# eazuooz/RayTracinginOneWeekendinCUDA

Hardware: AMD Instinct MI355X
Metric: Msamples/s (pixels x spp / s), whole job (higher is better)
Workload: dtype f64; 1 GPU; C2 Book-1 final random-spheres, HittableList world (no BVH), 1200x800x500spp x50 bounces; frames_in_flight=1, width=1200, height=800, spp=500, max_depth=50, seed=1984, variant=strict, rng=XORWOW (cuRAND device-API semantics), one sequence per pixel

## Files before the change

raytracinginoneweekendincuda_amd/csrc/device_scene.cpp:

```cpp
#include <hip/hip_runtime.h>

#include <cstdio>
#include <cmath>
#include <cstring>
#include <initializer_list>
#include <map>
#include <mutex>
#include <string>
#include <type_traits>
#include <utility>
#include <vector>

#include "../../include/rtow.h"
#include "device_arena.h"
#include "film_rows.h"
#include "launch_plan.h"
#include "primary_cull_rule.h"
#include "render_iface.h"
#include "scene_host.h"

namespace rtow {

static int hip_fail(hipError_t e, const char *what)
{
// ... 1004 lines not shown
    if (rc != RT_OK) {
        const std::string why = rt_last_error();
        hipStreamSynchronize(stream);
        mark_done(f);
        f.seeded = false;
        set_error(why);
        return rc;
    }
    f.last_samples = (uint64_t)f.geometry.n_pixels * (uint64_t)p->samples_per_pixel;
    f.last_variant = p->variant;
    f.last_adaptive = f.adaptive;
    f.last_direct = direct != nullptr;
    f.rendered = true;
    return RT_OK;
}

int rt_render_launch(rt_scene *scene, rt_film *film, const rt_render_params *p)
{
    if (int rc = frame_launch_check(scene, film, p, "rt_render_launch")) return rc;
    return launch_frame(scene, film, p, nullptr);
}

int rt_render_launch_direct(rt_scene *scene, rt_film *film, const rt_render_params *p, const rt_film_direct_params *direct)
{
    const std::string who = "rt_render_launch_direct";
    if (int rc = frame_launch_check(scene, film, p, who)) return rc;
    if (!direct) return fail(RT_ERR_INVALID, who + ": direct is NULL");
    if (direct->strategy != 0 && direct->strategy != 1) return fail(RT_ERR_INVALID, who + ": strategy must be 0 (uniform) or 1 (by area and brightness)");
    for (int32_t word : direct->reserved)
        if (word != 0) return fail(RT_ERR_INVALID, who + ": reserved must be 0");
    return launch_frame(scene, film, p, direct);
}

int rt_film_last_direct_stats(rt_film *film, rt_film_direct_stats *out)
{
    if (!film || !out) return fail(RT_ERR_INVALID, "rt_film_last_direct_stats: null argument");
    const FilmImpl &f = *F(film);
    if (!f.has_direct_stats) return fail(RT_ERR_STATE, "rt_film_last_direct_stats: no direct launch of this film has been finished");
    *out = f.direct_stats;
    return RT_OK;
}

void rt_film_direct_abi_sizes(uint32_t out2[2])
{
    out2[0] = (uint32_t)sizeof(rt_film_direct_params);
    out2[1] = (uint32_t)sizeof(rt_film_direct_stats);
}

#if RT_PHASES
static void print_phases(const FilmImpl &f)
{
    const unsigned long long *c = f.host_counters;
    const char *name[24] = {"node step", "leaf test", "shade", "refill", "  group/instance", "  medium", "  primitive", "",
                            "    record+xforms", "    box", "    sub-BVH", "    other geometry", "between walks again", "limited node pass", "node visits (lanes)", "",
                            "box pass", "medium pass / between walks", "object pass", "primitive pass", "  hit record", "  scatter",
                            "  next camera ray", "  pixel done"};
    if (is_sphere_list_kernel(f.last_kernel.kind)) {
        name[0] = "scan, pixel-parallel";
        name[1] = "scan, cooperative";
        name[12] = name[13] = "";
        const double passes = (double)c[96 + 0], groups = (double)c[96 + 12], taken = (double)c[64 + 12];
        if (groups > 0) {
            std::fprintf(stderr, "survivors: %.0f passes, %.2f groups of 4 per pass, groups taken f = %.4f\n", passes, groups / passes, taken / groups);
            std::fprintf(stderr, "survivors: spheres with a passing lane per taken group %.3f, lane appends per pass %.1f, lanes behind per pass %.2f\n",
                         (double)c[32 + 12] / taken, (double)c[96 + 13] / passes, (double)c[64 + 13] / passes);
            std::fprintf(stderr, "survivors: drains per pass %.2f, drain iterations (wave max of count) per pass %.2f, drain cycles %.1f %% of the "
                         "pixel-parallel scan's (%.0f of %.0f per pass)\n", (double)c[96 + 15] / passes, (double)c[64 + 15] / passes,
                         100.0 * c[32 + 13] / c[32 + 0], (double)c[32 + 13] / passes, (double)c[32 + 0] / passes);
        }
        name[19] = "";
        if (c[96 + 19])
            std::fprintf(stderr, "camera rays: %llu pixel-parallel passes, %.2f live lanes per pass, %.2f of them with a camera ray (depth 0): share %.4f\n",
                         c[96 + 19], (double)c[64 + 19] / c[96 + 19], (double)c[32 + 19] / c[96 + 19], (double)c[32 + 19] / (double)c[64 + 19]);
        name[23] = "";
        if (c[96 + 23])
            std::fprintf(stderr, "primary: %llu rounds, %.2f fresh lanes per round, %.2f list entries tested per round (%.2f per lane), %.0f cycles per round "
                         "(%.1f %% of wave time)\n", c[96 + 23], (double)c[64 + 23] / c[96 + 23], (double)c[32 + 15] / c[96 + 23],
                         (double)c[32 + 15] / (double)c[64 + 23], (double)c[32 + 23] / c[96 + 23], 100.0 * c[32 + 23] / (double)c[7]);
        name[14] = name[7] = "";
        if (c[96 + 7])
            std::fprintf(stderr, "window: %llu windowed passes (%llu windowed runs), %.2f trips scanned per pass in them, %.2f ranges per pass, %.0f cycles "
                         "of window computation per pass\n", c[96 + 7] * 16ull, c[96 + 14] * 16ull, (double)c[64 + 14] / c[96 + 7], (double)c[64 + 7] / c[96 + 7],
                         (double)c[32 + 14] / c[96 + 7]);
        name[16] = name[17] = name[18] = "";
        const double gp = (double)c[96 + 16];
        if (gp > 0) {
            std::fprintf(stderr, "grouped: %.0f passes through the filter, %.2f rays per pass, exact-test blocks executed per pass %.2f\n", gp,
                         (double)c[64 + 16] / gp, (double)c[32 + 16] / gp);
            std::fprintf(stderr, "grouped: survivors (lanes tested) per pass %.2f, largest per-lane count per pass %.2f, drains per pass %.2f\n",
                         (double)c[32 + 17] / gp, (double)c[64 + 17] / gp, (double)c[96 + 17] / gp);
            std::fprintf(stderr, "grouped: cycles per pass: filter %.0f, exact tests %.0f (%.1f %% and %.1f %% of the cooperative scans' %.0f)\n",
                         (double)c[64 + 18] / gp, (double)c[32 + 18] / gp, 100.0 * c[64 + 18] / c[32 + 1], 100.0 * c[32 + 18] / c[32 + 1],
                         (double)c[32 + 1] / (double)c[96 + 1]);
        }
    }
    const double total = (double)c[7];
    for (int k = 0; k < 24; k++)
        if (name[k][0] && c[96 + k])
            std::fprintf(stderr, "phase %-20s: %5.1f %% of wave time, %10llu passes, %5.1f lanes/pass, %7.0f cycles/pass\n", name[k],
                         100.0 * c[32 + k] / total, c[96 + k], (double)c[64 + k] / c[96 + k], (double)c[32 + k] / c[96 + k]);
}
#endif

int rt_render_finish(rt_scene *scene, rt_film *film, rt_render_stats *stats)
{
    (void)scene;
    if (!film) return fail(RT_ERR_INVALID, "rt_render_finish: null film");
    FilmImpl &f = *F(film);
    if (!f.in_flight) return fail(RT_ERR_STATE, "rt_render_finish: nothing launched");
    if (int rc = select_device(f.device)) return rc;
    const hipError_t waited = hipEventSynchronize(f.ev[3]);
    if (waited != hipSuccess && f.last_stream) hipStreamSynchronize(f.last_stream);
    mark_done(f);
    if (waited != hipSuccess) return hip_fail(waited, "hipEventSynchronize(render finished)");
    if (f.last_direct) {
        f.direct_stats = rt_film_direct_stats{f.host_counters[kShadowCounterWord], f.host_counters[kShadowCounterWord + 1], (uint32_t)f.last_direct_scratch, 0u};
        f.has_direct_stats = true;
    }
    if (stats) {
        std::memset(stats, 0, sizeof *stats);
        float ms_seed = 0, ms_render = 0;
        HIP_TRY(hipEventElapsedTime(&ms_seed, f.ev[0], f.ev[1]));
        HIP_TRY(hipEventElapsedTime(&ms_render, f.ev[1], f.ev[2]));
        const unsigned long long rays = f.host_counters[0];
#if RT_PHASES
        print_phases(f);
#endif
        stats->samples = f.last_adaptive ? (uint64_t)f.host_counters[2] : f.last_samples;
        stats->rays = rays;
        stats->seconds_seed = ms_seed * 1e-3;
        stats->seconds_render = ms_render * 1e-3;
        stats->pixels = f.geometry.n_pixels;
        stats->rows = (uint32_t)f.geometry.rows_owned;
        stats->kernel_vgprs = (uint32_t)f.last_kernel.vgprs;
        stats->lds_bytes = (uint32_t)f.last_kernel.lds_bytes;
        stats->kernel_kind = (uint32_t)f.last_kernel.kind;
        stats->pixels_per_wave = (uint32_t)f.last_plan.pixels_per_wave;
    }
    return RT_OK;
}

int rt_film_download(rt_film *film, double *frame_full, int width, int height)
{
    if (!film || !frame_full) return fail(RT_ERR_INVALID, "rt_film_download: null argument");
    FilmImpl &f = *F(film);
    if (width != f.geometry.width || height != f.geometry.height) return fail(RT_ERR_INVALID, "rt_film_download: frame size mismatch");
    if (int rc = select_device(f.device)) return rc;
    return download_rows(f, f.pixels, 3, false, frame_full);
}

int rt_film_set_adaptive(rt_film *film, const rt_adaptive_params *params)
{
    if (!film) return fail(RT_ERR_INVALID, "rt_film_set_adaptive: null film");
    FilmImpl &f = *F(film);
    if (f.in_flight) return fail(RT_ERR_STATE, "rt_film_set_adaptive: a render is in flight");
    if (params && !rule_in_range(*params))
        return fail(RT_ERR_INVALID, "rt_film_set_adaptive: needs min_samples >= 2, check_interval >= 1, noise_threshold >= 0, luminance_floor > 0");
    f.adaptive = params != nullptr;
    if (params) f.rule = to_rule(*params);
    return RT_OK;
}

int rt_film_download_sample_counts(rt_film *film, uint32_t *counts_full, int width, int height)
{
    if (!film || !counts_full) return fail(RT_ERR_INVALID, "rt_film_download_sample_counts: null argument");
    FilmImpl &f = *F(film);
    if (width != f.geometry.width || height != f.geometry.height) return fail(RT_ERR_INVALID, "rt_film_download_sample_counts: frame size mismatch");
    if (f.in_flight) return fail(RT_ERR_STATE, "rt_film_download_sample_counts: a render is in flight");
    if (int rc = select_device(f.device)) return rc;
    if (f.rendered && f.last_adaptive) return download_rows(f, f.ad_n, 1, true, counts_full);
    const std::vector<uint32_t> compact((size_t)f.geometry.n_pixels, f.rendered ? (uint32_t)f.frame_spp : 0u);
    scatter_owned_rows(compact.data(), 1, width, height, f.stripe_rows, f.rank, f.world_size, true, counts_full);
    return RT_OK;
}

int rt_film_download_probe_costs(rt_film *film, uint32_t *costs_full, int width, int height)
// ... 959 lines not shown
```

raytracinginoneweekendincuda_amd/csrc/render.hip:

```cpp
#include <hip/hip_runtime.h>

#include <cfloat>
#include <cstddef>
#include <cstdint>
#include <type_traits>

#include "flat_scene.h"
#include "launch_plan.h"
#include "primary_cull_rule.h"
#include "scan_window_rule.h"
#include "render_iface.h"
#include "rng.h"

#ifndef RT_STRICT
#define RT_STRICT 1
#endif
#ifndef RT_GROUP
#define RT_GROUP 0
#endif
#ifndef RT_ADAPT
#define RT_ADAPT 0
#endif
#ifndef RT_FEATURES
#define RT_FEATURES 0
// ... 324 lines not shown
            accept = aa_inside<P, Q>(f.wa, f.qp, f.qq, f.ku, f.kv, r, t[k]);                                            \
        }                                                                                                               \
        const bool take = live && accept;                                                                               \
        closest = take ? t[k] : closest;                                                                                \
        ref_best = take ? make_ref(REF_QUAD, quad_first + k) : ref_best;                                                \
        any = any || take;                                                                                              \
    }
    RT_BOX_FACE(0, 0, 1)
    RT_BOX_FACE(1, 2, 1)
    RT_BOX_FACE(2, 0, 1)
    RT_BOX_FACE(3, 2, 1)
    RT_BOX_FACE(4, 0, 2)
    RT_BOX_FACE(5, 0, 2)
#undef RT_BOX_FACE
    t_best = closest;
    return any;
}

DEV Vec msphere_center(const MSphereGeom &g, double tm, bool unit_time = false)
{
    double frac = unit_time ? tm : (tm - g.t0) / g.dt;
    return mk(g.c0x, g.c0y, g.c0z) + frac * mk(g.dcx, g.dcy, g.dcz);
}

DEV bool prim_test(const DeviceScene &sc, uint32_t ref, const Ray &r, double a, double tmin, double tmax, double &t)
{
    uint32_t idx = ref & kRefIndexMask;
    switch (ref >> kRefShift) {
    case REF_SPHERE: {
        SphereGeom g = sc.lds_spheres_tab != kNone ? lds_row<SphereGeom>(sc.lds_spheres_tab, idx) : const_row(sc.spheres, idx);
        return sphere_test(r.o - mk(g.cx, g.cy, g.cz), r.d, a, g.r2, tmin, tmax, t);
    }
    case REF_MSPHERE: {
        MSphereGeom g = const_row(sc.mspheres, idx);
        return sphere_test(r.o - msphere_center(g, r.tm, (sc.flags & SCENE_MS_UNIT_TIME) != 0), r.d, a, g.r2, tmin, tmax, t);
    }
    default: {
        return quad_test_at(sc, idx, r, tmin, tmax, t);
    }
    }
}

#ifndef RT_PHASES
#define RT_PHASES 0
#endif
#if RT_PHASES && RT_LANE_UNIT
#undef RT_PHASES
#define RT_PHASES 0
#endif
#if RT_PHASES
#define PH_BEGIN() const unsigned long long ph_t0 = __builtin_readcyclecounter()
#define PH_END(k, cond)                                                   \
    do {                                                                  \
        ph.t[k] += __builtin_readcyclecounter() - ph_t0;                  \
        ph.l[k] += (unsigned long long)__popcll(__ballot(cond));          \
        ph.n[k] += 1ull;                                                  \
    } while (0)
struct PhaseSums {
    unsigned long long t[24], l[24], n[24];
};
#define PH_ARG , PhaseSums &ph
#define PH_PASS , ph
#define PH_SUB_BEGIN() const unsigned long long ph_s0 = __builtin_readcyclecounter()
#define PH_COUNT(k) do { ph.l[k] += 1024ull; ph.n[k] += 1024ull; } while (0)
#define PH_SUB_END(k)                                                                              \
    do {                                                                                           \
        const unsigned long long ph_pc = (unsigned long long)__popcll(__ballot(true));             \
        ph.t[k] += (__builtin_readcyclecounter() - ph_s0) * 1024ull / ph_pc;                       \
        ph.l[k] += 1024ull;                                                                        \
        ph.n[k] += 1024ull / ph_pc;                                                                \
    } while (0)
#else
#define PH_BEGIN() do { } while (0)
#define PH_END(k, cond) do { } while (0)
#define PH_ARG
#define PH_PASS
#define PH_SUB_BEGIN() do { } while (0)
#endif
#if RT_PHASES
struct ScanSums {
    uint32_t groups, taken, spheres, appends, behind;
    uint32_t drains, drain_iters, drain_cycles;
    uint32_t win_runs, win_trips, win_ranges, win_cycles;
};
#define SS_ARG , ScanSums &ss
#define SS_PASS , ss
struct GroupedSums {
    uint32_t rays, tests, survivors, lane_max;
    uint32_t drains, filter_cycles, test_cycles;
};
#define GS_ARG , GroupedSums &gs
#define GS_PASS , gs
#else
#define SS_ARG
#define SS_PASS
#define GS_ARG
#define GS_PASS
#define PH_COUNT(k) do { } while (0)
#define PH_SUB_END(k) do { } while (0)
#endif
DEV Vec affine_rows(const DeviceScene &sc, uint32_t row, Vec p)
{
    const Xform r0 = get_xform(sc, row), r1 = get_xform(sc, row + 1), r2 = get_xform(sc, row + 2);
    return mk(((r0.a * p.x) + (r0.b * p.y)) + (r0.c * p.z), ((r1.a * p.x) + (r1.b * p.y)) + (r1.c * p.z), ((r2.a * p.x) + (r2.b * p.y)) + (r2.c * p.z));
}
DEV void affine_to_local(const DeviceScene &sc, uint32_t head, const Xform &x, Ray &lr)
{
    lr.o = affine_rows(sc, head + 4, lr.o - mk(x.a, x.b, x.c));
    lr.d = affine_rows(sc, head + 4, lr.d);
}
DEV void affine_to_world(const DeviceScene &sc, uint32_t head, Vec &p, Vec &n)
{
    const Xform t = get_xform(sc, head);
    p = affine_rows(sc, head + 1, p) + mk(t.a, t.b, t.c);
    const Xform i0 = get_xform(sc, head + 4), i1 = get_xform(sc, head + 5), i2 = get_xform(sc, head + 6);
    const Vec m = mk(((i0.a * n.x) + (i1.a * n.y)) + (i2.a * n.z), ((i0.b * n.x) + (i1.b * n.y)) + (i2.b * n.z), ((i0.c * n.x) + (i1.c * n.y)) + (i2.c * n.z));
    n = (1.0 / sqrt(length_sq(m))) * m;
}
struct MovingPose { Vec l[3], i[3], t; };
struct VecPair { Vec a, b; };
DEV MovingPose moving_pose(const Xform *rows, double tm)
{
    const Xform t0 = rows[0], dt = rows[4], key = rows[8];
    double s = (tm - key.a) / key.b;
    s = fmin(fmax(s, 0.0), 1.0);
    MovingPose m;
    for (uint32_t r = 0; r < 3; r++) {
        const Xform a = rows[1 + r], d = rows[5 + r];
        m.l[r] = mk(a.a + (s * d.a), a.b + (s * d.b), a.c + (s * d.c));
    }
    m.t = mk(t0.a + (s * dt.a), t0.b + (s * dt.b), t0.c + (s * dt.c));
    const Vec l0 = m.l[0], l1 = m.l[1], l2 = m.l[2];
    const double c00 = (l1.y * l2.z) - (l1.z * l2.y), c01 = (l1.z * l2.x) - (l1.x * l2.z), c02 = (l1.x * l2.y) - (l1.y * l2.x);
    const double c10 = (l0.z * l2.y) - (l0.y * l2.z), c11 = (l0.x * l2.z) - (l0.z * l2.x), c12 = (l0.y * l2.x) - (l0.x * l2.y);
    const double c20 = (l0.y * l1.z) - (l0.z * l1.y), c21 = (l0.z * l1.x) - (l0.x * l1.z), c22 = (l0.x * l1.y) - (l0.y * l1.x);
    const double det = ((l0.x * c00) + (l0.y * c01)) + (l0.z * c02);
    m.i[0] = mk(c00 / det, c10 / det, c20 / det);
    m.i[1] = mk(c01 / det, c11 / det, c21 / det);
    m.i[2] = mk(c02 / det, c12 / det, c22 / det);
    return m;
}
DEV Vec pose_rows(const Vec (&m)[3], Vec p)
{
    return mk(((m[0].x * p.x) + (m[0].y * p.y)) + (m[0].z * p.z), ((m[1].x * p.x) + (m[1].y * p.y)) + (m[1].z * p.z), ((m[2].x * p.x) + (m[2].y * p.y)) + (m[2].z * p.z));
}
DEV VecPair moving_local(const Xform *rows, double tm, Vec o, Vec d)
{
    const MovingPose m = moving_pose(rows, tm);
    return VecPair{pose_rows(m.i, o - m.t), pose_rows(m.i, d)};
}
DEV VecPair moving_world(const Xform *rows, double tm, Vec p, Vec n)
{
    const MovingPose m = moving_pose(rows, tm);
    const Vec v = mk(((m.i[0].x * n.x) + (m.i[1].x * n.y)) + (m.i[2].x * n.z), ((m.i[0].y * n.x) + (m.i[1].y * n.y)) + (m.i[2].y * n.z), ((m.i[0].z * n.x) + (m.i[1].z * n.y)) + (m.i[2].z * n.z));
    return VecPair{pose_rows(m.l, p) + m.t, (1.0 / sqrt(length_sq(v))) * v};
}
DEV const Xform *xform_rows(const DeviceScene &sc, uint32_t i)
{
    return (sc.lds_xforms != kNone ? reinterpret_cast<const Xform *>(lds_raw + sc.lds_xforms) : sc.xforms) + i;
}
DEV void moving_to_local(const DeviceScene &sc, uint32_t head, Ray &lr)
{
    const VecPair v = moving_local(xform_rows(sc, head), lr.tm, lr.o, lr.d);
    lr.o = v.a;
    lr.d = v.b;
}
// ... 1273 lines not shown
DEV ScanWindowSeg load_scan_window(const ScanWindowSeg *table, uint32_t k)
{
    const RT_CONST uint32_t *p = (const RT_CONST uint32_t *)(uintptr_t)(table + k);
    return ScanWindowSeg{p[0], __builtin_bit_cast(float, p[1]), __builtin_bit_cast(float, p[2]), p[3]};
}
DEV ScanTripSpan load_scan_span(const DeviceScene &sc, uint32_t t)
{
    if (sc.lds_scan_spans != kNone && sc.lds_scan_spans != 0u) {
        const v2f v = *(const RT_LDS v2f *)(lds_raw + sc.lds_scan_spans + t * (uint32_t)sizeof(ScanTripSpan));
        return ScanTripSpan{v.x, v.y};
    }
    return reinterpret_cast<const ScanTripSpan *>(sc.scan_segments + 2u * sc.n_scan_segments)[t];
}
template <int CTRL, int ROW_MASK>
DEV void fmin_step(float &x, float &y)
{
    const float ox = __builtin_bit_cast(float, __builtin_amdgcn_update_dpp(__builtin_bit_cast(int, x), __builtin_bit_cast(int, x), CTRL, ROW_MASK, 0xf, false));
    const float oy = __builtin_bit_cast(float, __builtin_amdgcn_update_dpp(__builtin_bit_cast(int, y), __builtin_bit_cast(int, y), CTRL, ROW_MASK, 0xf, false));
    x = __builtin_fminf(x, ox);
    y = __builtin_fminf(y, oy);
}
DEV void wave_fmin2(float &x, float &y)
{
    fmin_step<0xB1, 0xf>(x, y);
    fmin_step<0x4E, 0xf>(x, y);
    fmin_step<0x114, 0xf>(x, y);
    fmin_step<0x118, 0xf>(x, y);
    fmin_step<0x142, 0xa>(x, y);
    fmin_step<0x143, 0xc>(x, y);
    x = __builtin_bit_cast(float, __builtin_amdgcn_readlane(__builtin_bit_cast(int, x), 63));
    y = __builtin_bit_cast(float, __builtin_amdgcn_readlane(__builtin_bit_cast(int, y), 63));
}
template <bool ROWS_IN_LDS, bool WINDOWS>
DEV bool scan_filtered32(const DeviceScene &sc, bool live, uint32_t planes_off, uint32_t n_padded, uint16_t *queue, uint32_t lane,
                         const Ray &r, double tmin, double tmax, HitInfo &best SS_ARG)
{
    static_assert(kFilterTrip == 2 * kScanTripPairs && kScanAheadPairs == 2, "one trip = four pairs in two halves; set A of the next trip is read ahead");
    constexpr uint32_t kPairBytes = (uint32_t)sizeof(SphereScanPair), kTripBytes = kScanTripPairs * kPairBytes;
    const SphereScanPair *__restrict__ rows = sc.sphere_scan32;
    const ScanSegment *__restrict__ segments = sc.scan_segments;
    const SphereGeom *__restrict__ spheres = sc.spheres;
    const uint32_t n_segments = sc.n_scan_segments;
    const double a = dot(r.d, r.d);
    ScanRayPairs f = scan_ray_pairs(scan_ray32(r, a, sc.scan_reach32));
    if constexpr (WINDOWS)
        if (!live) f.nt = v2f{-__builtin_inff(), -__builtin_inff()};
    double closest = tmax;
    uint32_t best_k = kNone, count = 0;
    if (n_segments) {
        SphereScanPair a0 = load_scan_pair(rows, 0u, 0u), a1 = load_scan_pair(rows, 0u, kPairBytes);
        uint32_t off = 0, end = 0;
        for (uint32_t seg = 0; seg != n_segments; seg++) {
            const ScanSegment sg = load_scan_segment(segments, seg);
            end = (sg.first_trip + sg.n_trips) * kTripBytes;
            if (sg.axis == kScanAxisNone) {
                do scan_trip<false, ROWS_IN_LDS>(rows, spheres, off, end, a0, a1, f, f.ux, f.nt, planes_off, n_padded, queue, lane, count, r, a, tmin, closest, best_k SS_PASS);
                while (off != end);
            } else {
                const uint32_t seg_end = end;
                bool windowed = false;
                float x0 = 0.0f, x1 = 0.0f;
                uint32_t chunk = sg.first_trip;
                unsigned long long need = 0;
                if constexpr (WINDOWS) {
                    const ScanWindowSeg *windows = reinterpret_cast<const ScanWindowSeg *>(segments + n_segments);
                    const ScanWindowSeg ws = load_scan_window(windows, seg);
                    const uint32_t window_axis = ws.axis;
                    windowed = window_axis != kScanAxisNone;
                    if (windowed) {
#if RT_PHASES
                        const unsigned long long ss_w0 = __builtin_readcyclecounter();
#endif
                        const bool in_run = lane < sg.n_trips;
                        ScanTripSpan sp{0.0f, 0.0f};
                        if (in_run) sp = load_scan_span(sc, sg.first_trip + lane);
                        float e0 = __builtin_inff(), e1 = __builtin_inff();
                        if (live) {
                            const double oa = sg.axis == 0u ? r.o.x : (sg.axis == 1u ? r.o.y : r.o.z), da = sg.axis == 0u ? r.d.x : (sg.axis == 1u ? r.d.y : r.d.z);
                            const double ow = window_axis == 0u ? r.o.x : (window_axis == 1u ? r.o.y : r.o.z), dw = window_axis == 0u ? r.d.x : (window_axis == 1u ? r.d.y : r.d.z);
                            const ScanExtent ex = scan_window_extent(oa, da, ow, dw, __builtin_fabs(r.o.x) + __builtin_fabs(r.o.y) + __builtin_fabs(r.o.z), a, sc.scan_reach32, (double)ws.slab_lo, (double)ws.slab_hi);
                            e0 = (float)ex.lo;
                            e1 = -(float)ex.hi;
                        }
                        wave_fmin2(e0, e1);
                        x0 = e0;
                        x1 = -e1;
                        need = scan_window_fill(__ballot(in_run && scan_window_needs(sp.lo, sp.hi, x0, x1)));
#if RT_PHASES
                        asm volatile("" ::"s"(x0), "s"(x1));
                        ss.win_cycles += (uint32_t)(__builtin_readcyclecounter() - ss_w0);
                        ss.win_runs++;
#endif
                    }
                }
                if (sg.axis == 0u) { scan_swap(f.ux, f.uy); scan_swap(f.px, f.py); }
                if (sg.axis == 2u) { scan_swap(f.uz, f.uy); scan_swap(f.pz, f.py); }
                const v2f c = {sg.c, sg.c};
                v2f s0 = c * f.uy, l0 = __builtin_elementwise_fma(f.py, c, f.nt);
                if (!windowed) {
                    do scan_trip<true, ROWS_IN_LDS>(rows, spheres, off, end, a0, a1, f, s0, l0, planes_off, n_padded, queue, lane, count, r, a, tmin, closest, best_k SS_PASS);
                    while (off != end);
                } else {
                    for (;;) {
                        while (!need && (chunk + 64u) * kTripBytes < seg_end) {
                            chunk += 64u;
                            const uint32_t n = seg_end / kTripBytes - chunk;
                            bool mine = false;
                            if (lane < n) {
                                const ScanTripSpan sp = load_scan_span(sc, chunk + lane);
                                mine = scan_window_needs(sp.lo, sp.hi, x0, x1);
                            }
                            need = scan_window_fill(__ballot(mine));
                        }
                        if (!need) break;
                        const uint32_t first = (uint32_t)__builtin_ctzll(need);
                        const unsigned long long behind = ~(need >> first);
                        const uint32_t len = behind ? (uint32_t)__builtin_ctzll(behind) : 64u - first;
                        need &= need + (1ull << first);
                        const uint32_t start = (chunk + first) * kTripBytes;
                        if (start != off) {
                            off = start;
                            a0 = load_scan_pair(rows, off, 0u);
                            a1 = load_scan_pair(rows, off, kPairBytes);
                        }
                        end = start + len * kTripBytes;
#if RT_PHASES
                        ss.win_ranges++;
                        ss.win_trips += len;
#endif
                        do scan_trip<true, ROWS_IN_LDS>(rows, spheres, off, end, a0, a1, f, s0, l0, planes_off, n_padded, queue, lane, count, r, a, tmin, closest, best_k SS_PASS);
                        while (off != end);
                    }
                }
                if (off != seg_end) {
                    off = seg_end;
                    a0 = load_scan_pair(rows, off, 0u);
                    a1 = load_scan_pair(rows, off, kPairBytes);
                }
                if (sg.axis == 0u) { scan_swap(f.ux, f.uy); scan_swap(f.px, f.py); }
                if (sg.axis == 2u) { scan_swap(f.uz, f.uy); scan_swap(f.pz, f.py); }
            }
        }
    }
    drain_filtered<ROWS_IN_LDS>(spheres, planes_off, n_padded, queue, lane, count, r, a, tmin, closest, best_k SS_PASS);
    if (best_k == kNone) return false;
    best.t = closest;
    best.ref = make_ref(REF_SPHERE, best_k);
    best.obj = kNone;
    return true;
}

template <bool ROWS_IN_LDS>
DEV bool scan_filtered(const DeviceScene &sc, uint32_t planes_off, uint32_t n_padded, uint16_t *queue, uint32_t lane, const Ray &r, double tmin,
                       double tmax, HitInfo &best SS_ARG)
{
    const SphereScanRow *__restrict__ rows = sc.sphere_scan;
    const SphereGeom *__restrict__ spheres = sc.spheres;
    const uint32_t n = sc.n_spheres;
    const uint32_t n8 = n & ~7u;
    const double a = dot(r.d, r.d);
    const ScanRay f = scan_ray(r, a, sc.scan_reach);
    double closest = tmax;
    uint32_t best_k = kNone, count = 0;
    SphereScanRow a0{}, a1{}, a2{}, a3{};
    if (n8) {
        a0 = load_scan_row(rows, 0); a1 = load_scan_row(rows, 1);
        a2 = load_scan_row(rows, 2); a3 = load_scan_row(rows, 3);
    }
    for (uint32_t k0 = 0; k0 < n8; k0 += 8) {
        scan_rows_arrived(a0, a1, a2, a3);
        const SphereScanRow b0 = load_scan_row(rows, k0 + 4), b1 = load_scan_row(rows, k0 + 5);
        const SphereScanRow b2 = load_scan_row(rows, k0 + 6), b3 = load_scan_row(rows, k0 + 7);
        filter_four(a0, a1, a2, a3, k0, f, queue, lane, count);
        const uint32_t kn = (k0 + 8 < n8) ? k0 + 8 : k0;
// ... 127 lines not shown
                    const double cx = sv.plane(0, k), cy = sv.plane(1, k), cz = sv.plane(2, k);
                    const double fs = filter_s(f, cx, cy, cz);
                    q[u] = filter_q(f, fs, cx, cy, cz);
                    pass[u] = q[u] > sv.plane(4, k);
                }
#pragma unroll
                for (int u = 0; u < 4; u++) {
                    const uint32_t k = base + 64u * u + lane;
                    if (k < sv.n && pass[u]) {
                        double t;
                        if (sphere_test(r.o - mk(sv.plane(0, k), sv.plane(1, k), sv.plane(2, k)), r.d, a, sv.plane(3, k), tmin, bt, t)) {
                            bt = t;
                            bk = k;
                        }
                    }
                }
            }
        } else if (sv.in_lds) {
            for (uint32_t base = 0; base < sv.n_padded; base += 256u) {
                double b[4], c[4], disc[4];
#pragma unroll
                for (int u = 0; u < 4; u++) {
                    uint32_t k = base + 64u * u + lane;
                    k = k < sv.n_padded ? k : sv.n_padded - 1u;
                    Vec oc = r.o - mk(sv.plane(0, k), sv.plane(1, k), sv.plane(2, k));
                    b[u] = dot(oc, r.d);
                    c[u] = dot(oc, oc) - sv.plane(3, k);
                    disc[u] = b[u] * b[u] - a * c[u];
                }
#pragma unroll
                for (int u = 0; u < 4; u++) {
                    const uint32_t k = base + 64u * u + lane;
                    if (k < sv.n && disc[u] > 0.0 && !(b[u] > 0.0 && c[u] > 0.0)) {
                        double t;
                        if (sphere_roots(b[u], disc[u], a, tmin, bt, t)) {
                            bt = t;
                            bk = k;
                        }
                    }
                }
            }
        } else {
            for (uint32_t k = lane; k < sv.n; k += 64u) {
                SphereGeom g = sv.global[k];
                Vec oc = r.o - mk(g.cx, g.cy, g.cz);
                double b = dot(oc, r.d);
                double c = dot(oc, oc) - g.r2;
                double disc = b * b - a * c;
                if (disc > 0.0 && !(b > 0.0 && c > 0.0)) {
                    double t;
                    if (sphere_roots(b, disc, a, tmin, bt, t)) {
                        bt = t;
                        bk = k;
                    }
                }
            }
        }
        wave_min(bt, bk);
        if ((int)lane == src) {
            hit = bk != kNone;
            best.t = bt;
            best.ref = make_ref(REF_SPHERE, bk);
            best.obj = kNone;
        }
    }
}

DEV int lane_read(int v, int src_lane) { return __builtin_amdgcn_ds_bpermute(src_lane << 2, v); }
DEV double lane_read(double x, int src_lane)
{
    int lo = lane_read(__double2loint(x), src_lane);
    int hi = lane_read(__double2hiint(x), src_lane);
    return __hiloint2double(hi, lo);
}
DEV void min_with_lane(double &t, uint32_t &k, int partner)
{
    double ot = lane_read(t, partner);
    uint32_t ok = (uint32_t)lane_read((int)k, partner);
    bool take = (ot < t) || (ot == t && ok < k);
    t = take ? ot : t;
    k = take ? ok : k;
}

DEV void scan_grouped(const SphereView &sv, uint32_t lane, unsigned long long todo, const Ray &ray, double tmin, double tmax,
                      HitInfo &best, bool &hit GS_ARG)
{
    const int L = __popcll(todo);
    int log2m = 0;
    while ((1 << log2m) < L) log2m++;
    const int log2g = 6 - log2m;
    const uint32_t g = 1u << log2g;
    const uint32_t q = lane >> log2g, s = lane & (g - 1u);
    int owner = todo ? __ffsll((long long)todo) - 1 : (int)lane;
    {
        unsigned long long m = todo;
        for (int r = 0; r < L; r++) {
            const int src = __ffsll((long long)m) - 1;
            m &= m - 1;
            owner = q == (uint32_t)r ? src : owner;
        }
    }
    Ray r;
    r.o = mk(lane_read(ray.o.x, owner), lane_read(ray.o.y, owner), lane_read(ray.o.z, owner));
    r.d = mk(lane_read(ray.d.x, owner), lane_read(ray.d.y, owner), lane_read(ray.d.z, owner));
    const double a = dot(r.d, r.d);
    double bt = tmax;
    uint32_t bk = kNone;
    if (!sv.exact && sv.pairs_off) {
        const ScanRayPairs f = scan_ray_pairs(scan_ray32(r, a, sv.reach32));
        const uint32_t n_pairs = sv.n_padded / 2u;
        const v4f *rows = reinterpret_cast<const v4f *>(lds_raw + sv.pairs_off);
#if RT_PHASES
        uint32_t gs_mine = 0;
        gs.rays = (uint32_t)L;
#endif
        for (uint32_t base = 0; base < n_pairs; base += 2u * g) {
            v2f fs[2], fq[2], fk[2];
#if RT_PHASES
            const unsigned long long gs_t0 = __builtin_readcyclecounter();
#endif
#pragma unroll
            for (int h = 0; h < 2; h++) {
                uint32_t j = base + g * h + s;
                j = j < n_pairs ? j : n_pairs - 1u;
                const v4f lo = rows[j], hi = rows[n_pairs + j];
                const v2f cx = {lo.x, lo.y}, cy = {lo.z, lo.w}, cz = {hi.x, hi.y};
                fk[h] = v2f{hi.z, hi.w};
                fs[h] = __builtin_elementwise_fma(cz, f.uz, __builtin_elementwise_fma(cy, f.uy, cx * f.ux));
                fq[h] = __builtin_elementwise_fma(fs[h], fs[h], __builtin_elementwise_fma(f.pz, cz, __builtin_elementwise_fma(f.py, cy, __builtin_elementwise_fma(f.px, cx, f.nt))));
            }
            const float sv4[4] = {fs[0].x, fs[0].y, fs[1].x, fs[1].y}, qv4[4] = {fq[0].x, fq[0].y, fq[1].x, fq[1].y};
            const float kv4[4] = {fk[0].x, fk[0].y, fk[1].x, fk[1].y};
#if RT_PHASES
            const unsigned long long gs_t1 = __builtin_readcyclecounter();
#pragma unroll
            for (int u = 0; u < 4; u++) {
                const bool tested = 2u * (base + g * (uint32_t)(u >> 1) + s) + (uint32_t)(u & 1) < sv.n && qv4[u] > kv4[u];
                const unsigned long long m = __ballot(tested);
                gs.tests += m ? 1u : 0u;
                gs.survivors += (uint32_t)__popcll(m);
                gs_mine += tested ? 1u : 0u;
            }
            const unsigned long long gs_t2 = __builtin_readcyclecounter();
            gs.filter_cycles += (uint32_t)(gs_t1 - gs_t0);
#endif
#pragma unroll
            for (int u = 0; u < 4; u++) {
                const uint32_t k = 2u * (base + g * (uint32_t)(u >> 1) + s) + (uint32_t)(u & 1);
                if (k < sv.n && qv4[u] > kv4[u]) {
                    const float bu = f.od - sv4[u];
                    const bool behind = bu > f.root_m && __builtin_fmaf(bu, bu, kv4[u] - qv4[u]) > 0.0f;
                    double t;
                    if (!behind && sphere_test(r.o - mk(sv.plane(0, k), sv.plane(1, k), sv.plane(2, k)), r.d, a, sv.plane(3, k), tmin, bt, t)) {
                        bt = t;
                        bk = k;
                    }
                }
            }
#if RT_PHASES
            asm volatile("" ::"v"(bt), "v"(bk));
            gs.test_cycles += (uint32_t)(__builtin_readcyclecounter() - gs_t2);
#endif
        }
#if RT_PHASES
        for (int off = 32; off > 0; off >>= 1) gs_mine = max(gs_mine, (uint32_t)__shfl_xor((int)gs_mine, off, 64));
        gs.lane_max = gs_mine;
#endif
    } else if (!sv.exact) {
        const ScanRay f = scan_ray(r, a, sv.reach);
#if RT_PHASES
        uint32_t gs_mine = 0;
        gs.rays = (uint32_t)L;
#endif
        for (uint32_t base = 0; base < sv.n_padded; base += 4u * g) {
            bool pass[4];
#if RT_PHASES
            const unsigned long long gs_t0 = __builtin_readcyclecounter();
#endif
#pragma unroll
            for (int u = 0; u < 4; u++) {
                uint32_t k = base + g * u + s;
                k = k < sv.n_padded ? k : sv.n_padded - 1u;
                const double cx = sv.plane(0, k), cy = sv.plane(1, k), cz = sv.plane(2, k);
                const double fs = filter_s(f, cx, cy, cz);
                pass[u] = filter_q(f, fs, cx, cy, cz) > sv.plane(4, k);
            }
#if RT_PHASES
            const unsigned long long gs_t1 = __builtin_readcyclecounter();
#pragma unroll
            for (int u = 0; u < 4; u++) {
                const bool tested = base + g * u + s < sv.n && pass[u];
                const unsigned long long m = __ballot(tested);
                gs.tests += m ? 1u : 0u;
                gs.survivors += (uint32_t)__popcll(m);
                gs_mine += tested ? 1u : 0u;
            }
            const unsigned long long gs_t2 = __builtin_readcyclecounter();
            gs.filter_cycles += (uint32_t)(gs_t1 - gs_t0);
#endif
#pragma unroll
            for (int u = 0; u < 4; u++) {
                const uint32_t k = base + g * u + s;
                if (k < sv.n && pass[u]) {
                    double t;
                    if (sphere_test(r.o - mk(sv.plane(0, k), sv.plane(1, k), sv.plane(2, k)), r.d, a, sv.plane(3, k), tmin, bt, t)) {
                        bt = t;
                        bk = k;
                    }
                }
            }
#if RT_PHASES
            asm volatile("" ::"v"(bt), "v"(bk));
            gs.test_cycles += (uint32_t)(__builtin_readcyclecounter() - gs_t2);
#endif
        }
#if RT_PHASES
        for (int off = 32; off > 0; off >>= 1) gs_mine = max(gs_mine, (uint32_t)__shfl_xor((int)gs_mine, off, 64));
        gs.lane_max = gs_mine;
#endif
    } else
    for (uint32_t base = 0; base < sv.n_padded; base += 4u * g) {
        double b[4], c[4], disc[4];
#pragma unroll
        for (int u = 0; u < 4; u++) {
            uint32_t k = base + g * u + s;
            k = k < sv.n_padded ? k : sv.n_padded - 1u;
            Vec oc = r.o - mk(sv.plane(0, k), sv.plane(1, k), sv.plane(2, k));
            b[u] = dot(oc, r.d);
            c[u] = dot(oc, oc) - sv.plane(3, k);
            disc[u] = b[u] * b[u] - a * c[u];
        }
#pragma unroll
        for (int u = 0; u < 4; u++) {
            const uint32_t k = base + g * u + s;
            if (k < sv.n && disc[u] > 0.0 && !(b[u] > 0.0 && c[u] > 0.0)) {
                double t;
                if (sphere_roots(b[u], disc[u], a, tmin, bt, t)) {
                    bt = t;
                    bk = k;
                }
            }
        }
    }
    if (log2g >= 1) min_step<0xB1, 0xf>(bt, bk);
    if (log2g >= 2) min_step<0x4E, 0xf>(bt, bk);
    if (log2g >= 3) min_step<0x141, 0xf>(bt, bk);
    if (log2g >= 4) min_step<0x140, 0xf>(bt, bk);
    if (log2g >= 5) min_with_lane(bt, bk, (int)lane ^ 16);
    if (log2g >= 6) min_with_lane(bt, bk, (int)lane ^ 32);
// ... 1029 lines not shown
                        todo = freshes;
                        if (!fresh) n_listed = 0u;
                        n_listed = n_listed < kPrimaryListMax ? n_listed : kPrimaryListMax;
                        const double ra = dot(ray.d, ray.d);
                        double closest = DBL_MAX;
                        uint32_t best_k = kNone;
#if RT_PHASES
                        ph.n[23] += 1ull;
                        ph.l[23] += (unsigned long long)__popcll(freshes);
                        for (uint32_t e = n_listed, off = 32; off > 0; off >>= 1) {
                            e += (uint32_t)__shfl_xor((int)e, (int)off, 64);
                            if (off == 1) ph.t[15] += e;
                        }
#endif
                        for (uint32_t s = 0; __any(s < n_listed); s++) {
                            if (s == 7u) {
                                if (s < n_listed) wa = row[1];
                            } else {
                                wa.x = __builtin_amdgcn_alignbit(wa.y, wa.x, 16); wa.y = __builtin_amdgcn_alignbit(wa.z, wa.y, 16);
                                wa.z = __builtin_amdgcn_alignbit(wa.w, wa.z, 16); wa.w >>= 16;
                            }
                            if (s < n_listed) {
                                const uint32_t k = wa.x & 0xFFFFu;
                                SphereGeom g;
                                if (sv.in_lds) {
                                    const RT_LDS double *pl = (const RT_LDS double *)(lds_raw + sv.planes_off);
                                    g = SphereGeom{pl[k], pl[sv.n_padded + k], pl[2u * sv.n_padded + k], pl[3u * sv.n_padded + k]};
                                } else {
                                    g = sc.spheres[k];
                                }
                                double t;
                                if (sphere_test(ray.o - mk(g.cx, g.cy, g.cz), ray.d, ra, g.r2, 0.001, closest, t)) {
                                    closest = t;
                                    best_k = k;
                                }
                            }
                        }
                        hit = best_k != kNone;
                        if (hit) {
                            h.t = closest;
                            h.ref = make_ref(REF_SPHERE, best_k);
                            h.obj = kNone;
                        }
                    }
#if RT_PHASES
                    if (primary_last) {
                        asm volatile("" ::"v"(h.t), "v"(h.ref));
                        ph.t[23] += __builtin_readcyclecounter() - ph_t0;
                    }
#endif
                }
            }
            if (primary_last) {
            } else if (scan_wave) {
                primary_since_scan = false;
                PH_BEGIN();
#if RT_PHASES
                ScanSums ss{};
#endif
                if (a.exact_scan || a.filter_fp64) {
                    if (active) hit = a.exact_scan ? scan_uniform(sc, queue, lane, ray, 0.001, DBL_MAX, h)
                                      : sv.in_lds  ? scan_filtered<true>(sc, sv.planes_off, sv.n_padded, queue, lane, ray, 0.001, DBL_MAX, h SS_PASS)
                                                   : scan_filtered<false>(sc, 0u, 0u, queue, lane, ray, 0.001, DBL_MAX, h SS_PASS);
                } else if (a.scan_windows) {
                    hit = sv.in_lds ? scan_filtered32<true, true>(sc, active, sv.planes_off, sv.n_padded, queue, lane, ray, 0.001, DBL_MAX, h SS_PASS)
                                    : scan_filtered32<false, true>(sc, active, 0u, 0u, queue, lane, ray, 0.001, DBL_MAX, h SS_PASS);
                } else {
                    if (active) hit = sv.in_lds ? scan_filtered32<true, false>(sc, true, sv.planes_off, sv.n_padded, queue, lane, ray, 0.001, DBL_MAX, h SS_PASS)
                                                : scan_filtered32<false, false>(sc, true, 0u, 0u, queue, lane, ray, 0.001, DBL_MAX, h SS_PASS);
                }
                PH_END(0, active);
#if RT_PHASES
                ph.n[19] += 1ull;
                ph.l[19] += (unsigned long long)__popcll(live);
                ph.t[19] += (unsigned long long)__popcll(__ballot(active && depth == 0));
                {
                    const int src = __ffsll((long long)__ballot(active)) - 1;
                    if (src >= 0) {
                    const auto rl = [src](uint32_t v) { return (unsigned long long)(uint32_t)__builtin_amdgcn_readlane((int)v, src); };
                    ph.n[12] += rl(ss.groups);  ph.l[12] += rl(ss.taken);        ph.t[12] += rl(ss.spheres);
                    ph.n[13] += rl(ss.appends); ph.l[13] += rl(ss.behind);       ph.t[13] += rl(ss.drain_cycles);
                    ph.n[15] += rl(ss.drains);  ph.l[15] += rl(ss.drain_iters);
                    ph.n[14] += rl(ss.win_runs); ph.l[14] += rl(ss.win_trips);   ph.t[14] += rl(ss.win_cycles);
                    ph.n[7] += rl(ss.win_runs) ? 1ull : 0ull; ph.l[7] += rl(ss.win_ranges);
                    }
                }
#endif
            } else {
                PH_BEGIN();
#if RT_PHASES
                GroupedSums gs{};
#endif
                if (sv.in_lds && !a.coop_single) scan_grouped(sv, lane, todo, ray, 0.001, DBL_MAX, h, hit GS_PASS);
                else scan_cooperative(sv, lane, todo, ray, 0.001, DBL_MAX, h, hit);
                PH_END(1, (todo >> lane) & 1ull);
#if RT_PHASES
                if (gs.rays) {
                    ph.n[16] += 1ull;       ph.l[16] += gs.rays;     ph.t[16] += gs.tests;
                    ph.n[17] += gs.drains;  ph.l[17] += gs.lane_max; ph.t[17] += gs.survivors;
                    ph.l[18] += gs.filter_cycles; ph.t[18] += gs.test_cycles;
                }
#endif
            }
        }
        bool thin = false;
        if constexpr (T::WORLD == 0 && !T::COMPOSITE) {
            thin = sc.ms_planes != nullptr && exhausted && __popcll(live) < a.coop_threshold;
            if (thin) {
                PH_BEGIN();
                scan_grouped_ms(sc, lane, live, ray, 0.001, DBL_MAX, h, hit);
                walk.state = kNone;
                PH_END(1, active);
            }
        }
        if constexpr (T::WORLD == 0) if (!thin) {
            const int n_rounds = T::BATCH ? a.rounds : (T::COMPOSITE ? kRoundsComposite : (T::FAST ? kRoundsFast : kRounds));
            for (int round = 0; round < n_rounds; round++) {
                if constexpr (T::SEG) {
                    const bool between = active && walk.state == kNone && seg.hi != kSegEnd;
                    if (__any(between)) {
                        PH_BEGIN();
#if RT_PHASES
                        const bool ph_again = between && seg.hi != 0u;
#endif
                        if (between) seg_advance<T>(sc, ray, walk, walk_best, rng, seg PH_PASS);
                        PH_END(17, between);
#if RT_PHASES
                        if (__any(ph_again)) PH_END(12, ph_again);
#endif
                    }
                }
                for (int step = 0; step < (T::COMPOSITE ? a.node_burst : kBurst); step++) {
                    const bool mover = walk_moving(walk.state);
                    [[maybe_unused]] bool limited_walks = false;
                    if constexpr (T::SEG) limited_walks = __any(mover && seg.hi != kSegEnd);
                    const int movers = __popcll(__ballot(mover));
                    const int parked = __popcll(__ballot(walk_parked(walk.state)));
                    if (movers == 0 || movers * (T::COMPOSITE ? a.park_ratio : 1) < parked) break;
                    {
                        PH_BEGIN();
#if RT_PHASES
                        if (limited_walks) PH_END(13, mover && seg.hi != kSegEnd);
#endif
                        if (mover) {
                            if constexpr (T::FAST) {
                                walk_node_fast(ray, 0.001, walk);
                                PH_COUNT(14);
                                if (walk_moving(walk.state)) {
                                    walk_node_fast(ray, 0.001, walk);
                                    PH_COUNT(14);
                                }
                            } else if constexpr (T::SEG) {
                                if (limited_walks) {
                                    walk_node_seg(sc, ray, 0.001, walk, seg.hi);
                                    PH_COUNT(14);
                                    if (walk_moving(walk.state)) {
                                        walk_node_seg(sc, ray, 0.001, walk, seg.hi);
                                        PH_COUNT(14);
                                    }
                                } else {
                                    walk_node_open(ray, 0.001, walk);
                                    PH_COUNT(14);
                                    if (walk_moving(walk.state)) {
                                        walk_node_open(ray, 0.001, walk);
                                        PH_COUNT(14);
                                    }
                                }
                            } else
                            {
                                walk_node<T::BATCH>(nv, ray, 0.001, walk);
                                PH_COUNT(14);
                            }
                            if constexpr ((!T::COMPOSITE || T::BATCH) && !T::FAST && !T::SEG) {
                                if (walk_moving(walk.state)) {
                                    walk_node<T::BATCH>(nv, ray, 0.001, walk);
                                    PH_COUNT(14);
// ... 2357 lines not shown
```

Measured before the change: 3497 Msamples/s.

## Queue grouped-scan filter survivors and drain exact sphere tests in batches

The grouped cooperative scan used to run the exact double-precision sphere test inline, under per-lane divergence, right after each float filter step. It now ballots the filter results, skips blocks where no lane survives, and appends surviving sphere indices to a per-lane LDS queue. That queue is drained in batches with the existing drain_filtered routine, which should keep the f64 tests more convergent across the wave. In exchange it adds queue writes, extra drain passes and LDS pressure. It also adds profiling-only counters for window lane-trips and grouped drains.

```diff
diff --git a/raytracinginoneweekendincuda_amd/csrc/device_scene.cpp b/raytracinginoneweekendincuda_amd/csrc/device_scene.cpp
--- a/raytracinginoneweekendincuda_amd/csrc/device_scene.cpp
+++ b/raytracinginoneweekendincuda_amd/csrc/device_scene.cpp
@@ -1110,6 +1110,9 @@
             std::fprintf(stderr, "window: %llu windowed passes (%llu windowed runs), %.2f trips scanned per pass in them, %.2f ranges per pass, %.0f cycles "
                          "of window computation per pass\n", c[96 + 7] * 16ull, c[96 + 14] * 16ull, (double)c[64 + 14] / c[96 + 7], (double)c[64 + 7] / c[96 + 7],
                          (double)c[32 + 14] / c[96 + 7]);
+        if (c[96 + 7])
+            std::fprintf(stderr, "window: %.1f lane-trips per windowed pass by each lane's own extent (sum over the live lanes), %.2f a live lane\n",
+                         (double)c[32 + 7] / c[96 + 7], c[64 + 19] ? (double)c[32 + 7] / c[96 + 7] / ((double)c[64 + 19] / c[96 + 19]) : 0.0);
         name[16] = name[17] = name[18] = "";
         const double gp = (double)c[96 + 16];
         if (gp > 0) {
@@ -1120,6 +1123,8 @@
             std::fprintf(stderr, "grouped: cycles per pass: filter %.0f, exact tests %.0f (%.1f %% and %.1f %% of the cooperative scans' %.0f)\n",
                          (double)c[64 + 18] / gp, (double)c[32 + 18] / gp, 100.0 * c[64 + 18] / c[32 + 1], 100.0 * c[32 + 18] / c[32 + 1],
                          (double)c[32 + 1] / (double)c[96 + 1]);
+            std::fprintf(stderr, "grouped: appends per pass %.2f, drains per pass %.2f, drain iterations per pass %.2f\n", (double)c[32 + 17] / gp,
+                         (double)c[96 + 17] / gp, (double)c[32 + 16] / gp);
         }
     }
     const double total = (double)c[7];
diff --git a/raytracinginoneweekendincuda_amd/csrc/render.hip b/raytracinginoneweekendincuda_amd/csrc/render.hip
--- a/raytracinginoneweekendincuda_amd/csrc/render.hip
+++ b/raytracinginoneweekendincuda_amd/csrc/render.hip
@@ -430,6 +430,7 @@
     uint32_t groups, taken, spheres, appends, behind;
     uint32_t drains, drain_iters, drain_cycles;
     uint32_t win_runs, win_trips, win_ranges, win_cycles;
+    uint32_t win_lane_trips;
 };
 #define SS_ARG , ScanSums &ss
 #define SS_PASS , ss
@@ -1869,6 +1870,9 @@
                             e0 = (float)ex.lo;
                             e1 = -(float)ex.hi;
                         }
+#if RT_PHASES
+                        const float own0 = e0, own1 = -e1;
+#endif
                         wave_fmin2(e0, e1);
                         x0 = e0;
                         x1 = -e1;
@@ -1877,6 +1881,10 @@
                         asm volatile("" ::"s"(x0), "s"(x1));
                         ss.win_cycles += (uint32_t)(__builtin_readcyclecounter() - ss_w0);
                         ss.win_runs++;
+                        for (uint32_t t = 0; t < sg.n_trips; t++) {
+                            const ScanTripSpan own = load_scan_span(sc, sg.first_trip + t);
+                            ss.win_lane_trips += (uint32_t)__popcll(__ballot(live && scan_window_needs(own.lo, own.hi, own0, own1)));
+                        }
 #endif
                     }
                 }
@@ -2170,7 +2178,7 @@
     k = take ? ok : k;
 }
 
-DEV void scan_grouped(const SphereView &sv, uint32_t lane, unsigned long long todo, const Ray &ray, double tmin, double tmax,
+DEV void scan_grouped(const SphereView &sv, uint16_t *queue, uint32_t lane, unsigned long long todo, const Ray &ray, double tmin, double tmax,
                       HitInfo &best, bool &hit GS_ARG)
 {
     const int L = __popcll(todo);
@@ -2198,20 +2206,23 @@
         const ScanRayPairs f = scan_ray_pairs(scan_ray32(r, a, sv.reach32));
         const uint32_t n_pairs = sv.n_padded / 2u;
         const v4f *rows = reinterpret_cast<const v4f *>(lds_raw + sv.pairs_off);
+        uint32_t count = 0;
 #if RT_PHASES
+        ScanSums ss{};
         uint32_t gs_mine = 0;
         gs.rays = (uint32_t)L;
+        const unsigned long long gs_t0 = __builtin_readcyclecounter();
 #endif
         for (uint32_t base = 0; base < n_pairs; base += 2u * g) {
             v2f fs[2], fq[2], fk[2];
-#if RT_PHASES
-            const unsigned long long gs_t0 = __builtin_readcyclecounter();
-#endif
+            uint32_t jj[2];
+            bool on[2];
 #pragma unroll
             for (int h = 0; h < 2; h++) {
-                uint32_t j = base + g * h + s;
-                j = j < n_pairs ? j : n_pairs - 1u;
-                const v4f lo = rows[j], hi = rows[n_pairs + j];
+                const uint32_t j = base + g * h + s;
+                on[h] = j < n_pairs;
+                jj[h] = on[h] ? j : n_pairs - 1u;
+                const v4f lo = rows[jj[h]], hi = rows[n_pairs + jj[h]];
                 const v2f cx = {lo.x, lo.y}, cy = {lo.z, lo.w}, cz = {hi.x, hi.y};
                 fk[h] = v2f{hi.z, hi.w};
                 fs[h] = __builtin_elementwise_fma(cz, f.uz, __builtin_elementwise_fma(cy, f.uy, cx * f.ux));
@@ -2219,40 +2230,32 @@
             }
             const float sv4[4] = {fs[0].x, fs[0].y, fs[1].x, fs[1].y}, qv4[4] = {fq[0].x, fq[0].y, fq[1].x, fq[1].y};
             const float kv4[4] = {fk[0].x, fk[0].y, fk[1].x, fk[1].y};
-#if RT_PHASES
-            const unsigned long long gs_t1 = __builtin_readcyclecounter();
+            const bool p[4] = {on[0] && qv4[0] > kv4[0], on[0] && qv4[1] > kv4[1], on[1] && qv4[2] > kv4[2], on[1] && qv4[3] > kv4[3]};
+            const unsigned long long m[4] = {__ballot(p[0]), __ballot(p[1]), __ballot(p[2]), __ballot(p[3])};
+            if (__builtin_expect((m[0] | m[1] | m[2] | m[3]) != 0, 0)) {
 #pragma unroll
-            for (int u = 0; u < 4; u++) {
-                const bool tested = 2u * (base + g * (uint32_t)(u >> 1) + s) + (uint32_t)(u & 1) < sv.n && qv4[u] > kv4[u];
-                const unsigned long long m = __ballot(tested);
-                gs.tests += m ? 1u : 0u;
-                gs.survivors += (uint32_t)__popcll(m);
-                gs_mine += tested ? 1u : 0u;
-            }
-            const unsigned long long gs_t2 = __builtin_readcyclecounter();
-            gs.filter_cycles += (uint32_t)(gs_t1 - gs_t0);
-#endif
-#pragma unroll
-            for (int u = 0; u < 4; u++) {
-                const uint32_t k = 2u * (base + g * (uint32_t)(u >> 1) + s) + (uint32_t)(u & 1);
-                if (k < sv.n && qv4[u] > kv4[u]) {
+                for (int u = 0; u < 4; u++) {
+                    if (!m[u]) continue;
                     const float bu = f.od - sv4[u];
                     const bool behind = bu > f.root_m && __builtin_fmaf(bu, bu, kv4[u] - qv4[u]) > 0.0f;
-                    double t;
-                    if (!behind && sphere_test(r.o - mk(sv.plane(0, k), sv.plane(1, k), sv.plane(2, k)), r.d, a, sv.plane(3, k), tmin, bt, t)) {
-                        bt = t;
-                        bk = k;
-                    }
-                }
-            }
 #if RT_PHASES
-            asm volatile("" ::"v"(bt), "v"(bk));
-            gs.test_cycles += (uint32_t)(__builtin_readcyclecounter() - gs_t2);
-#endif
-        }
+                    gs.survivors += (uint32_t)__popcll(__ballot(p[u] && !behind));
+                    gs_mine += p[u] && !behind ? 1u : 0u;
+#endif
+                    append_survivor(queue, lane, count, 2u * jj[u >> 1] + (uint32_t)(u & 1), p[u] && !behind);
+                }
+                if (__any(count > (uint32_t)(kQueueCap - 4))) drain_filtered<true>(sv.global, sv.planes_off, sv.n_padded, queue, lane, count, r, a, tmin, bt, bk SS_PASS);
+            }
+        }
+        drain_filtered<true>(sv.global, sv.planes_off, sv.n_padded, queue, lane, count, r, a, tmin, bt, bk SS_PASS);
 #if RT_PHASES
+        asm volatile("" ::"v"(bt), "v"(bk));
         for (int off = 32; off > 0; off >>= 1) gs_mine = max(gs_mine, (uint32_t)__shfl_xor((int)gs_mine, off, 64));
         gs.lane_max = gs_mine;
+        gs.drains = ss.drains;
+        gs.tests = ss.drain_iters;
+        gs.test_cycles = ss.drain_cycles;
+        gs.filter_cycles = (uint32_t)(__builtin_readcyclecounter() - gs_t0) - ss.drain_cycles;
 #endif
     } else if (!sv.exact) {
         const ScanRay f = scan_ray(r, a, sv.reach);
@@ -3448,7 +3451,7 @@
                     ph.n[13] += rl(ss.appends); ph.l[13] += rl(ss.behind);       ph.t[13] += rl(ss.drain_cycles);
                     ph.n[15] += rl(ss.drains);  ph.l[15] += rl(ss.drain_iters);
                     ph.n[14] += rl(ss.win_runs); ph.l[14] += rl(ss.win_trips);   ph.t[14] += rl(ss.win_cycles);
-                    ph.n[7] += rl(ss.win_runs) ? 1ull : 0ull; ph.l[7] += rl(ss.win_ranges);
+                    ph.n[7] += rl(ss.win_runs) ? 1ull : 0ull; ph.l[7] += rl(ss.win_ranges); ph.t[7] += rl(ss.win_lane_trips);
                     }
                 }
 #endif
@@ -3457,7 +3460,7 @@
 #if RT_PHASES
                 GroupedSums gs{};
 #endif
-                if (sv.in_lds && !a.coop_single) scan_grouped(sv, lane, todo, ray, 0.001, DBL_MAX, h, hit GS_PASS);
+                if (sv.in_lds && !a.coop_single) scan_grouped(sv, queue, lane, todo, ray, 0.001, DBL_MAX, h, hit GS_PASS);
                 else scan_cooperative(sv, lane, todo, ray, 0.001, DBL_MAX, h, hit);
                 PH_END(1, (todo >> lane) & 1ull);
 #if RT_PHASES
```

Result: faster. 3607 Msamples/s (median of 6 runs) (+3.2%).
